# Dzh-16/FLASH-Viterbi

Hardware: AMD Instinct MI355X
Metric: trellis_cells_per_sec (higher is better)
Workload: dtype f32 scores (+f64 add per cell, rounded to f32 as the reference does)

## Files before the change

flash_viterbi_amd/csrc/fv_full.hip:

```cpp
#include "fv_internal.h"
#include "fv_kernels.hip.inc"
#include "flashvit_testing.h"

namespace {

int pick_kernel(const fv_ctx *ctx)
{
    if (ctx->opt_kernel == FV_KERNEL_F64_STREAM) return FV_KERNEL_F64_STREAM;
    if (!ctx->view.logs_nonpositive) return FV_KERNEL_F64_STREAM;
    if (ctx->opt_kernel == FV_KERNEL_F16_REFINE || ctx->opt_kernel == FV_KERNEL_F32_REFINE ||
        ctx->opt_kernel == FV_KERNEL_Q16_REFINE || ctx->opt_kernel == FV_KERNEL_U16_REFINE)
        return ctx->opt_kernel;
    if (ctx->opt_kernel == FV_KERNEL_SPARSE_Q16) return ctx->SPdata.p ? FV_KERNEL_SPARSE_Q16 : FV_KERNEL_U16_REFINE;
    return (ctx->SPdata.p && ctx->density <= 0.35) ? FV_KERNEL_SPARSE_Q16 : FV_KERNEL_U16_REFINE;
}

constexpr int U_UP = 16, U_DB32 = 4, U_DB64 = 2, U_DB16 = 2;

constexpr int nb_slot(int NB) { return NB == 1 ? 0 : NB == 2 ? 1 : NB == 4 ? 2 : 3; }
template <typename TA> constexpr int tab_slot()
{
    return std::is_same<TA, double>::value ? 0 : std::is_same<TA, float>::value ? 1 : std::is_same<TA, fvk::half_t>::value ? 2 : 3;
}
template <typename TA, int NB, bool DB> constexpr unsigned long long step_variant()
{
    return 1ull << ((tab_slot<TA>() == 0 ? 0 : 4 + (tab_slot<TA>() - 1) * 6) + (DB ? 0 : 4) + nb_slot(NB));
}
template <typename TA> constexpr unsigned long long slab_variant() { return 1ull << (22 + tab_slot<TA>()); }
template <int NB, bool DB, int NWV> constexpr unsigned long long u16_variant()
{
    return 1ull << (26 + (NWV == 16 ? 0 : 8) + (DB ? 4 : 0) + nb_slot(NB));
}
template <int NB> constexpr unsigned long long sparse_variant() { return 1ull << (42 + nb_slot(NB)); }
template <int NB, bool MEM> constexpr unsigned long long csr_variant() { return 1ull << (FV_TV_CSR_SHIFT + (MEM ? 4 : 0) + nb_slot(NB)); }
template <int NB, bool MEM> constexpr unsigned long long csr_f64_variant() { return (1ull << (FV_TV_CSR64_SHIFT + nb_slot(NB))) | (MEM ? 1ull << (FV_TV_CSR64_SHIFT + 4) : 0ull); }
static_assert(step_variant<double, 8, true>() == FV_TV_F64_NB8 && step_variant<float, 2, false>() == FV_TV_F32_UP_NB2 &&
              step_variant<fvk::half_t, 1, true>() == FV_TV_F16_NB1 && step_variant<fvk::q16_t, 2, false>() == FV_TV_Q16_UP_NB2 &&
// ... 258 lines not shown
}

int max_batch_for(int nrows, bool u16_only)
{
    if (u16_only) {
        if (fvk::u16_lds_bytes<8, 8>(nrows) <= 160 * 1024) return 8;
        if (fvk::u16_lds_bytes<4, 8>(nrows) <= 160 * 1024) return 4;
        if (fvk::u16_lds_bytes<2, 8>(nrows) <= 160 * 1024) return 2;
        return 1;
    }
    int nb = fvk::MAX_BATCH;
    while (nb > 1) {
        size_t need = nb == 8 ? fvk::step_lds_bytes<8>(nrows) : nb == 4 ? fvk::step_lds_bytes<4>(nrows)
                                                                        : fvk::step_lds_bytes<2>(nrows);
        if (need <= 160 * 1024) break;
        nb >>= 1;
    }
    return nb;
}

struct ProfRange { size_t first, count; };

int prof_event(fv_ctx *ctx, size_t idx, hipEvent_t *out)
{
    while (ctx->prof_events.size() <= idx) {
        hipEvent_t e;
        FV_HIP(hipEventCreate(&e));
        ctx->prof_events.push_back(e);
    }
    *out = ctx->prof_events[idx];
    return 0;
}

enum { BATCH_NONE = 0, BATCH_SERIAL = 1, BATCH_FORK = 2 };
int run_generation_full(fv_ctx *ctx, std::vector<fv::Pass> &passes, int kernel, size_t &nprof, int batch = BATCH_NONE)
{
    const int K = ctx->K;
    const int np = (int)passes.size();
    if (np == 0) return 0;
    std::stable_sort(passes.begin(), passes.end(),
                     [](const fv::Pass &a, const fv::Pass &b) { return a.R - a.L > b.R - b.L; });
    for (int base = 0; base < np; base += fvk::PASS_CHUNK) {
        fvk::PassChunk ch;
        ch.n = std::min(fvk::PASS_CHUNK, np - base);
        for (int q = 0; q < ch.n; ++q) {
            const fv::Pass &p = passes[base + q];
            ch.p[q] = fvk::PassDesc{ p.L, p.R, p.from_pi ? 1 : 0, p.whole ? 1 : 0, (long long)(base + q) * 2 * ctx->nrows };
        }
        if (ctx->csr)
            hipLaunchKernelGGL(fvk::init_rows_csr, dim3((K + 255) / 256, ch.n), dim3(256), 0, ctx->stream, ch, ctx->CRptr.p,
                               ctx->CRcol.p, ctx->CRlog.p, ctx->view.lb64, ctx->LPi64.p, ctx->d_ob.p, ctx->d_ans.p, ctx->d_rows.p, K);
        else
        hipLaunchKernelGGL(fvk::init_rows, dim3((K + 255) / 256, ch.n), dim3(256), 0, ctx->stream, ch,
                           ctx->LA64.p, ctx->nrows, ctx->view.lb64, ctx->LPi64.p, ctx->d_ob.p, ctx->d_ans.p,
                           ctx->d_rows.p, K);
        FV_HIP(hipGetLastError());
    }
    const int maxlen = passes[0].R - passes[0].L;
    const bool slabbed = (kernel == FV_KERNEL_F64_STREAM || kernel == FV_KERNEL_Q16_REFINE) && !ctx->full_ok;
    int cap = std::max(1, std::min(ctx->opt_max_batch, slabbed ? 4 : max_batch_for(ctx->nrows, !ctx->full_ok)));
    if (kernel == FV_KERNEL_SPARSE_CSR || kernel == FV_KERNEL_CSR_F64) cap = ctx->opt_max_batch;
    const bool whole_gen = passes[0].whole;
    constexpr int FORK_STREAMS = 3, FORK_CAP = 4;
    const bool two = ((kernel == FV_KERNEL_U16_REFINE && ctx->u16_ok) || ((kernel == FV_KERNEL_SPARSE_Q16 || kernel == FV_KERNEL_SPARSE_CSR || kernel == FV_KERNEL_CSR_F64) && maxlen >= 64)) &&
                     !(ctx->opt_debug & 262144) && (!whole_gen || batch == BATCH_FORK) && np > FORK_CAP &&
                     !ctx->opt_profile && !(ctx->opt_debug & 64);
    const int nbatches = (np + FORK_CAP - 1) / FORK_CAP;
    const int nstreams = two ? std::min(FORK_STREAMS, nbatches) : 1;
    auto fork = [&]() -> int {
        FV_HIP(hipEventRecord(ctx->ev_fork, ctx->stream));
        for (int q = 1; q < nstreams; ++q) FV_HIP(hipStreamWaitEvent(ctx->aux[q - 1], ctx->ev_fork, 0));
        return 0;
    };
    if (two) {
        cap = std::min(cap, FORK_CAP);
        if (!ctx->fork_active) {
            hipError_t qe;
            while ((qe = hipStreamQuery(ctx->stream)) == hipErrorNotReady) std::this_thread::yield();
            FV_HIP(qe);
        }
        ctx->fork_active = true;
        { int rc = fork(); if (rc) return rc; }
    }
    ctx->forked_batches = two;
    struct Unfork { fv_ctx *c; ~Unfork() { c->forked_batches = false; c->lstream = nullptr; } } unfork{ ctx };
    auto join = [&]() -> int {
        for (int q = 1; q < nstreams; ++q) {
            FV_HIP(hipEventRecord(ctx->ev_join[q - 1], ctx->aux[q - 1]));
            FV_HIP(hipStreamWaitEvent(ctx->stream, ctx->ev_join[q - 1], 0));
        }
        return 0;
    };
    const bool col_last = !(ctx->opt_debug & 8);
    const bool use_graph = (ctx->opt_debug & 64) && !ctx->opt_profile;
    if (use_graph) FV_HIP(hipStreamBeginCapture(ctx->stream, hipStreamCaptureModeThreadLocal));
    if (whole_gen && !use_graph) FV_HIP(hipEventRecord(ctx->ev_s0, ctx->stream));
    int active = np;
    for (int s = 1; s <= maxlen; ++s) {
        while (active > 0 && passes[active - 1].R - passes[active - 1].L < s) --active;
        int full = active;
        if (col_last) while (full > 0 && passes[full - 1].R - passes[full - 1].L == s && !passes[full - 1].whole) --full;
        auto row = [&](int q, int parity) { return ctx->d_rows.p + (size_t)q * 2 * ctx->nrows + (size_t)parity * ctx->nrows; };
        for (int base = 0; base < full; base += cap) {
            const int nb = std::min(cap, full - base);
            fvk::TaskSlot slots[fvk::MAX_BATCH];
            for (int q = 0; q < nb; ++q) {
                const fv::Pass &p = passes[base + q];
                slots[q].t1_in = row(base + q, (s - 1) & 1);
                slots[q].t1_out = row(base + q, s & 1);
                slots[q].tmp_row = ctx->view.lb32 + (size_t)ctx->h_ob[p.L + s] * K;
                slots[q].tmp64_row = ctx->view.lb64 + (size_t)ctx->h_ob[p.L + s] * K;
                slots[q].bp_out = ctx->d_bp.p + (size_t)(p.L + s) * K;
            }
            hipEvent_t e0 = nullptr, e1 = nullptr;
            if (ctx->opt_profile) {
                int rc = prof_event(ctx, nprof, &e0); if (rc) return rc;
                rc = prof_event(ctx, nprof + 1, &e1); if (rc) return rc;
                nprof += 2;
                FV_HIP(hipEventRecord(e0, ctx->stream));
            }
            const int other = two ? (base / cap) % nstreams : 0;
            ctx->lstream = other ? ctx->aux[other - 1] : ctx->stream;
            int rc = launch_step_kernel(ctx, kernel, slots, nb, s & 1);
            ctx->lstream = nullptr;
            if (rc) return rc;
            if (ctx->opt_profile) FV_HIP(hipEventRecord(e1, ctx->stream));
            ctx->stats.step_launches += 1;
            ctx->stats.task_steps += nb;
        }
        for (int sid = 0; sid < nstreams; ++sid) {
            fvk::ColArgs c;
            c.LA64 = ctx->LA64.p; c.ans = ctx->d_ans.p; c.K = K; c.nrows = ctx->nrows; c.n = 0;
            hipStream_t cst = sid ? ctx->aux[sid - 1] : ctx->stream;
            auto flush = [&]() -> int {
                if (c.n == 0) return 0;
                if (ctx->csr) {
                    fvk::CsrColArgs cc;
                    cc.ck = ctx->CSk.p; cc.c64 = ctx->CS64.p; cc.tile_off = ctx->CSoff.p; cc.tile_nwb = ctx->CSnwb.p;
                    cc.ans = ctx->d_ans.p; cc.K = K; cc.n = c.n;
                    std::copy(c.p, c.p + c.n, cc.p);
                    hipLaunchKernelGGL(fvk::last_column_csr, dim3(c.n), dim3(256), 0, cst, cc);
                } else
                hipLaunchKernelGGL(fvk::last_column, dim3(c.n), dim3(256), 0, cst, c);
                FV_HIP(hipGetLastError());
                ctx->stats.column_steps += c.n;
                c.n = 0;
                return 0;
            };
            for (int q = full; q < active; ++q) {
                const int owner = (two && s > 1) ? (q / cap) % nstreams : 0;
                if (owner != sid) continue;
                const fv::Pass &p = passes[q];
                c.p[c.n++] = fvk::ColJob{ row(q, (s - 1) & 1), ctx->view.lb32 + (size_t)ctx->h_ob[p.R] * K, ctx->d_bp.p + (size_t)p.R * K, p.R };
                if (c.n == fvk::COL_CHUNK) { int rc = flush(); if (rc) return rc; }
            }
            int rc = flush();
            if (rc) return rc;
        }
    }
    if (use_graph) {
        hipGraph_t g = nullptr;
        FV_HIP(hipStreamEndCapture(ctx->stream, &g));
        hipGraphExec_t ge = nullptr;
        FV_HIP(hipGraphInstantiate(&ge, g, nullptr, nullptr, 0));
        if (whole_gen) FV_HIP(hipEventRecord(ctx->ev_s0, ctx->stream));
        FV_HIP(hipGraphLaunch(ge, ctx->stream));
        ctx->graphs.push_back(ge);
        (void)hipGraphDestroy(g);
    }
    if (whole_gen && !two) FV_HIP(hipEventRecord(ctx->ev_s1, ctx->stream));
    if (two) { int rc = join(); if (rc) return rc; }
    if (whole_gen && two) FV_HIP(hipEventRecord(ctx->ev_s1, ctx->stream));
    if (batch) {
        fvk::ArgmaxArgs a;
        a.rows = ctx->d_rows.p; a.ans = ctx->d_ans.p; a.score = ctx->d_score.p; a.K = K; a.nrows = ctx->nrows; a.n = 0;
        auto flush = [&]() -> int {
            if (a.n == 0) return 0;
            hipLaunchKernelGGL(fvk::final_argmax_batch, dim3(a.n), dim3(1024), 0, ctx->stream, a);
            FV_HIP(hipGetLastError());
            a.n = 0;
            return 0;
        };
        for (int q = 0; q < np; ++q) {
            if (!passes[q].whole) continue;
            const int len = passes[q].R - passes[q].L;
            a.j[a.n++] = fvk::ArgmaxJob{ q * 2 + (len & 1), passes[q].R, passes[q].seq };
            if (a.n == fvk::ARGMAX_CHUNK) { int rc = flush(); if (rc) return rc; }
        }
        int rc = flush();
        if (rc) return rc;
    }
    for (int q = 0; q < np && !batch; ++q) {
        if (!passes[q].whole) continue;
        const int len = passes[q].R - passes[q].L;
        const float *last = ctx->d_rows.p + (size_t)q * 2 * ctx->nrows + (size_t)(len & 1) * ctx->nrows;
        hipLaunchKernelGGL(fvk::final_argmax, dim3(1), dim3(1024), 0, ctx->stream, last, K,
                           ctx->d_ans.p + passes[q].R, ctx->d_score.p);
        FV_HIP(hipGetLastError());
    }
    for (int base = 0; base < np; base += fvk::PASS_CHUNK) {
        fvk::PassChunk ch;
        ch.n = std::min(fvk::PASS_CHUNK, np - base);
        for (int q = 0; q < ch.n; ++q) {
            const fv::Pass &p = passes[base + q];
            ch.p[q] = fvk::PassDesc{ p.L, p.R, p.from_pi ? 1 : 0, p.whole ? 1 : 0, 0 };
        }
        hipLaunchKernelGGL(fvk::backtrack, dim3(ch.n), dim3(64), 0, ctx->stream, ch, ctx->d_bp.p, K, ctx->d_ans.p);
        FV_HIP(hipGetLastError());
    }
    return 0;
}

}

namespace fvi {

int full_setup(fv_ctx *ctx)
{
    int rc = 0;
    if ((rc = allow_big_lds<float, 1>(ctx)) || (rc = allow_big_lds<float, 2>(ctx)) || (rc = allow_big_lds<float, 4>(ctx)) ||
        (rc = allow_big_lds<float, 8>(ctx)) || (rc = allow_big_lds<double, 1>(ctx)) || (rc = allow_big_lds<double, 2>(ctx)) ||
        (rc = allow_big_lds<double, 4>(ctx)) || (rc = allow_big_lds<double, 8>(ctx)) ||
        (rc = allow_big_lds<fvk::half_t, 1>(ctx)) || (rc = allow_big_lds<fvk::half_t, 2>(ctx)) ||
        (rc = allow_big_lds<fvk::half_t, 4>(ctx)) || (rc = allow_big_lds<fvk::half_t, 8>(ctx)) ||
        (rc = allow_big_lds<fvk::q16_t, 1>(ctx)) || (rc = allow_big_lds<fvk::q16_t, 2>(ctx)) ||
        (rc = allow_big_lds<fvk::q16_t, 4>(ctx)) || (rc = allow_big_lds<fvk::q16_t, 8>(ctx)) ||
        (rc = set_big_lds(ctx, &fvk::trellis_step_sparse<1>)) || (rc = set_big_lds(ctx, &fvk::trellis_step_sparse<2>)) ||
        (rc = set_big_lds(ctx, &fvk::trellis_step_sparse<4>)) || (rc = set_big_lds(ctx, &fvk::trellis_step_sparse<8>)))
        return rc;
    if ((rc = set_big_lds(ctx, &fvk::trellis_step_csr<1, false>)) || (rc = set_big_lds(ctx, &fvk::trellis_step_csr<2, false>)) ||
        (rc = set_big_lds(ctx, &fvk::trellis_step_csr<4, false>)) || (rc = set_big_lds(ctx, &fvk::trellis_step_csr<8, false>)))
        return rc;
// ... 124 lines not shown
        double lmax, dqmax;
        std::memcpy(&lmax, &bits[0], 8); std::memcpy(&dqmax, &bits[1], 8);
        const float stepf = lmax > 0.0 ? (float)(lmax / 65534.0) : 1.0f;
        ctx->windowq = std::nextafter((float)(2.0 * dqmax), HUGE_VALF);
        ctx->qscale = -stepf;
        ctx->laq16_ready = true;
    }
    return fvi::ensure_workspace(ctx, T, rows_needed, nscores);
}

void start_full_stats(fv_ctx *ctx, int kernel, int generations)
{
    long long table = (long long)((ctx->K + fvk::TILE_W - 1) / fvk::TILE_W) * ctx->nrows * fvk::TILE_W * (kernel == FV_KERNEL_F64_STREAM ? 8 : kernel == FV_KERNEL_F32_REFINE ? 4 : 2);
    if (kernel == FV_KERNEL_SPARSE_Q16) table = (long long)ctx->SPdata.bytes();
    if (kernel == FV_KERNEL_SPARSE_CSR) table = (long long)(ctx->CSk.bytes() + ctx->CSq.bytes());
    if (kernel == FV_KERNEL_CSR_F64) table = (long long)(ctx->CSk.bytes() + ctx->CS64.bytes());
    ctx->start_stats(kernel, generations, table, ctx->density);
}

int decode_full_impl(fv_ctx *ctx, const int *ob, int T, int n_split, int mode, int *path_out, float *score_out)
{
    if (!ctx || !path_out || T < 2 || n_split < 1) return FV_ERR_ARG;
    int rc = fvi::emission_view(ctx, ob, T);
    if (rc) return rc;
    if (ctx->K == 0) return FV_ERR_STATE;
    auto t0 = clk::now();
    fv::Plan plan;
    rc = fv::build_plan(T, n_split, mode, ctx->nranks, plan);
    if (rc) return rc;
    size_t most = 1;
    std::vector<std::vector<fv::Pass>> gens = fvi::deal_passes(ctx, plan, &most);
    int kernel = FV_KERNEL_AUTO;
    if ((rc = prepare_full(ctx, ob, T, most, kernel))) return rc;
    start_full_stats(ctx, kernel, plan.generations());

    if ((rc = fvi::begin_decode(ctx, ob, T))) return rc;
    FV_HIP(hipEventRecord(ctx->ev_start, ctx->stream));
    size_t nprof = 0;
    ctx->fork_active = false;
    for (size_t g = 0; g < gens.size(); ++g) {
        ctx->stats.passes += (int)gens[g].size();
        if ((rc = run_generation_full(ctx, gens[g], kernel, nprof))) return rc;
        if (g == 0) FV_HIP(hipEventRecord(ctx->ev_top, ctx->stream));
    }
    ctx->close_stats((long long)ctx->K * ctx->K, ctx->K);
    const long long whole[2] = { 0, T };
    return fvi::finish_decode(ctx, plan, whole, 1, path_out, score_out, nullptr, t0, nprof, false);
}

int decode_full_batch_impl(fv_ctx *ctx, const int *ob, const long long *offsets, int nseq, int n_split, int mode, int *path_out,
                           float *score_out, int *status_out)
{
    const char *who = "fv_decode_full_batch";
    std::vector<int> lengths;
    int rc = fvi::batch_lengths(ctx, who, ob, offsets, nseq, n_split, mode, path_out, lengths);
    if (rc || (rc = fvi::batch_symbols(ctx, who, ob, offsets, nseq))) return rc;
    auto t0 = clk::now();
    const int sumT = (int)offsets[nseq];
    fv::Plan plan;
    if ((rc = fvi::batch_plan(ctx, who, lengths, n_split, mode, plan))) return rc;
    size_t most = 1;
    std::vector<std::vector<fv::Pass>> gens = fvi::deal_passes(ctx, plan, &most);
    int kernel = FV_KERNEL_AUTO;
    if ((rc = prepare_full(ctx, ob, sumT, most, kernel, std::max(nseq, 2)))) return rc;
    start_full_stats(ctx, kernel, plan.generations());

    if ((rc = fvi::begin_decode(ctx, ob, sumT))) return rc;
    FV_HIP(hipEventRecord(ctx->ev_start, ctx->stream));
    size_t nprof = 0;
    ctx->fork_active = false;
    const int gen0 = (ctx->opt_debug & (1 << 28)) ? BATCH_SERIAL : BATCH_FORK;
    for (size_t g = 0; g < gens.size(); ++g) {
        ctx->stats.passes += (int)gens[g].size();
        if ((rc = run_generation_full(ctx, gens[g], kernel, nprof, gen0))) return rc;
        if (g == 0) FV_HIP(hipEventRecord(ctx->ev_top, ctx->stream));
    }
    ctx->close_stats((long long)ctx->K * ctx->K, ctx->K);
    return fvi::finish_decode(ctx, plan, offsets, nseq, path_out, score_out, status_out, t0, nprof, false);
}

int test_forward_impl(fv_ctx *ctx, const int *ob, int T, const fv_test_pass *tp, int np, float *rows_out, int *bp_out,
                      unsigned long long *variants_out)
{
    if (!tp || np < 1 || !rows_out || !bp_out || T < 2) return FV_ERR_ARG;
    if (int rv = fvi::emission_view(ctx, ob, T)) return rv;
    if (ctx->K == 0) return FV_ERR_STATE;
    const int K = ctx->K;
    std::vector<fv::Pass> gen((size_t)np);
    std::vector<int> byL((size_t)np);
    for (int q = 0; q < np; ++q) {
        const fv_test_pass &p = tp[q];
        if (p.L < 0 || p.R <= p.L || p.R >= T) { ctx->detail = "fv_test_forward: a pass needs 0 <= L < R < T"; return FV_ERR_ARG; }
        if (p.L == 0 ? p.init_state >= 0 : (p.init_state < 0 || p.init_state >= K)) {
            ctx->detail = "fv_test_forward: init_state < 0 (Pi) at L = 0 only, a state in [0, K) at L > 0";
            return FV_ERR_ARG;
        }
        gen[(size_t)q] = fv::Pass{ p.L, p.R, p.L == 0, false, 0, -1 };
        byL[(size_t)q] = q;
    }
    std::sort(byL.begin(), byL.end(), [&](int a, int b) { return tp[a].L < tp[b].L; });
    for (int q = 1; q < np; ++q)
        if (tp[byL[q]].L <= tp[byL[q - 1]].R) { ctx->detail = "fv_test_forward: passes overlap"; return FV_ERR_ARG; }
    int kernel = FV_KERNEL_AUTO;
    int rc = prepare_full(ctx, ob, T, (size_t)np, kernel);
    if (rc) return rc;
    start_full_stats(ctx, kernel, 1);
    ctx->stats.passes = np;
// ... 152 lines not shown
```

flash_viterbi_amd/csrc/fv_kernels.hip.inc:

```
#pragma once

#include <hip/hip_runtime.h>

#include <cfloat>
#include <climits>
#include <cstdint>
#include <type_traits>

#include "fv_device_common.h"

#ifdef FV_TIMING_BUILD
#define FV_TIMING_BIT(debug, bit) (((debug) & (bit)) != 0)
#else
#define FV_TIMING_BIT(debug, bit) false
#endif

namespace fvk {


struct TaskSlot {
    const float *t1_in;
    float *t1_out;
    int *bp_out;
    const float *tmp_row;
// ... 1329 lines not shown
        float r = m1[t];
        int kbest = k1[t];
        wave_best(r, kbest);
        if (lane < TILE_W) { redR[(t * TILE_W + c) * SP_WAVES + w] = r; redK[(t * TILE_W + c) * SP_WAVES + w] = kbest; }
    }
    __syncthreads();
    if (w < NB && w < args.nb) {
        float r = FV_NEG_INF;
        int kbest = INT_MAX;
        if (rg < 2) {
            const float4 fv = *reinterpret_cast<const float4 *>(redR + (w * TILE_W + c) * SP_WAVES + rg * 4);
            const int4 fk = *reinterpret_cast<const int4 *>(redK + (w * TILE_W + c) * SP_WAVES + rg * 4);
            r = fv.x; kbest = fk.x;
            if (better(fv.y, fk.y, r, kbest)) { r = fv.y; kbest = fk.y; }
            if (better(fv.z, fk.z, r, kbest)) { r = fv.z; kbest = fk.z; }
            if (better(fv.w, fk.w, r, kbest)) { r = fv.w; kbest = fk.w; }
        }
        wave_best(r, kbest);
        if (lane < TILE_W && col < K) {
            const bool any = r > -FLT_MAX;
            args.t[w].t1_out[col] = any ? r : -FLT_MAX;
            args.t[w].bp_out[col] = any ? kbest : -1;
        }
    }
}

template <int NB>
static inline size_t csr_f64_lds_bytes(int nrows, bool mem)
{
    return (mem ? (size_t)0 : (size_t)nrows * NB * 4) + (size_t)NB * SP_WAVES * TILE_W * 8;
}



__global__ void init_rows(const PassChunk ch, const double *LA64, int nrows, const double *LB64T,
                          const double *LPi64, const int *ob, const int *ans, float *rows, int K)
{
    const PassDesc p = ch.p[blockIdx.y];
    const int i = blockIdx.x * blockDim.x + threadIdx.x;
    if (i >= K) return;
    int st = p.from_pi ? -1 : ans[p.L - 1];
    const double x = st < 0 ? LPi64[i] : LA64[tab_index<4>(st, i, nrows)];
    rows[p.row_off + i] = (float)(x + LB64T[(size_t)ob[p.L] * K + i]);
}

__global__ __launch_bounds__(1024) void final_argmax(const float *row, int K, int *ans_last, float *score_out)
{
    __shared__ float sv[16];
    __shared__ int sk[16];
    float v = FV_NEG_INF;
    int k = INT_MAX;
    for (int i = threadIdx.x; i < K; i += blockDim.x) {
        const float x = row[i];
        if (x > v) { v = x; k = i; }
    }
#pragma unroll
    for (int m = 1; m < 64; m <<= 1) {
        float ov = __shfl_xor(v, m);
        int ok = __shfl_xor(k, m);
        if (better(ov, ok, v, k)) { v = ov; k = ok; }
    }
    const int lane = threadIdx.x & 63, w = threadIdx.x >> 6;
    if (lane == 0) { sv[w] = v; sk[w] = k; }
    __syncthreads();
    if (threadIdx.x == 0) {
        for (int q = 1; q < (int)(blockDim.x >> 6); ++q)
            if (better(sv[q], sk[q], v, k)) { v = sv[q]; k = sk[q]; }
        *ans_last = k;
        *score_out = v;
    }
}

struct ArgmaxJob { int row; int R; int seq; };
constexpr int ARGMAX_CHUNK = 256;
struct ArgmaxArgs { const float *rows; int *ans; float *score; int K, nrows, n; ArgmaxJob j[ARGMAX_CHUNK]; };

// ... 8 lines not shown
    int k = INT_MAX;
    for (int i = threadIdx.x; i < args.K; i += blockDim.x) {
        const float x = row[i];
        if (x > v) { v = x; k = i; }
    }
#pragma unroll
    for (int m = 1; m < 64; m <<= 1) {
        float ov = __shfl_xor(v, m);
        int ok = __shfl_xor(k, m);
        if (better(ov, ok, v, k)) { v = ov; k = ok; }
    }
    const int lane = threadIdx.x & 63, w = threadIdx.x >> 6;
    if (lane == 0) { sv[w] = v; sk[w] = k; }
    __syncthreads();
    if (threadIdx.x == 0) {
        for (int q = 1; q < (int)(blockDim.x >> 6); ++q)
            if (better(sv[q], sk[q], v, k)) { v = sv[q]; k = sk[q]; }
        args.ans[job.R] = k;
        args.score[job.seq] = v;
    }
}

struct ColJob { const float *t1_in; const float *tmp_row; int *bp_row; int R; };
constexpr int COL_CHUNK = 48;
struct ColArgs { const double *LA64; const int *ans; int K, nrows, n; ColJob p[COL_CHUNK]; };

__global__ __launch_bounds__(256) void last_column(const ColArgs args)
{
    __shared__ float sv[4];
    __shared__ int sk[4];
    const ColJob job = args.p[blockIdx.x];
    const int i = args.ans[job.R];
    if (i < 0 || i >= args.K) return;
    const float tmp = job.tmp_row[i];
    const double *col = args.LA64 + (size_t)(i >> 4) * args.nrows * TILE_W + (i & 15) * 4;
    float best = FV_NEG_INF;
    int arg = INT_MAX;
    for (int k0 = threadIdx.x; k0 < args.K; k0 += 256 * 4) {
        float t1[4];
        double L[4];
#pragma unroll
        for (int u = 0; u < 4; ++u) {
            const int k = k0 + 256 * u, ks = k < args.K ? k : 0;
            t1[u] = job.t1_in[ks];
            L[u] = col[(size_t)(ks >> 2) * (TILE_W * 4) + (ks & 3)];
        }
#pragma unroll
        for (int u = 0; u < 4; ++u) {
            const int k = k0 + 256 * u;
            if (k < args.K) {
                const float y = exact_cell(tmp, t1[u], L[u]);
                if (y > best) { best = y; arg = k; }
            }
        }
    }
#pragma unroll
    for (int m = 1; m < 64; m <<= 1) {
        const float ov = __shfl_xor(best, m);
        const int ok = __shfl_xor(arg, m);
        if (better(ov, ok, best, arg)) { best = ov; arg = ok; }
    }
    const int lane = threadIdx.x & 63, w = threadIdx.x >> 6;
    if (lane == 0) { sv[w] = best; sk[w] = arg; }
    __syncthreads();
    if (threadIdx.x == 0) {
        for (int q = 1; q < 4; ++q)
            if (better(sv[q], sk[q], best, arg)) { best = sv[q]; arg = sk[q]; }
        job.bp_row[i] = best > -FLT_MAX ? arg : -1;
    }
}

__global__ void init_rows_csr(const PassChunk ch, const long long *rptr, const int *rcol, const double *rlog,
                              const double *LB64T, const double *LPi64, const int *ob, const int *ans, float *rows, int K)
{
    const PassDesc p = ch.p[blockIdx.y];
    const int i = blockIdx.x * blockDim.x + threadIdx.x;
    if (i >= K) return;
    const int st = p.from_pi ? -1 : ans[p.L - 1];
    double x;
    if (st < 0) {
        x = LPi64[i];
    } else {
        long long lo = rptr[st], hi = rptr[st + 1];
        const long long end = hi;
        while (lo < hi) {
            const long long mid = lo + (hi - lo) / 2;
            if (rcol[mid] < i) lo = mid + 1; else hi = mid;
        }
        x = (lo < end && rcol[lo] == i) ? rlog[lo] : -__builtin_huge_val();
    }
    rows[p.row_off + i] = (float)(x + LB64T[(size_t)ob[p.L] * K + i]);
}

struct CsrColArgs {
    const uint4 *ck; const double *c64; const long long *tile_off; const int *tile_nwb;
    const int *ans; int K, n; ColJob p[COL_CHUNK];
};

__global__ __launch_bounds__(256) void last_column_csr(const CsrColArgs args)
{
    __shared__ float sv[4];
    __shared__ int sk[4];
    const ColJob job = args.p[blockIdx.x];
    const int i = args.ans[job.R];
    if (i < 0 || i >= args.K) return;
    const float tmp = job.tmp_row[i];
    const int tile = i >> 4, c = i & 15;
    const size_t v0 = (size_t)args.tile_off[tile] + c;
    const int nent = args.tile_nwb[tile] * 16;
    const unsigned int *kw = reinterpret_cast<const unsigned int *>(args.ck);
    float best = FV_NEG_INF;
    int arg = INT_MAX;
    for (int n0 = threadIdx.x; n0 < nent; n0 += 256 * 4) {
        float t1[4];
        double L[4];
        int ks[4];
#pragma unroll
        for (int u = 0; u < 4; ++u) {
            const int n = n0 + 256 * u, ns = n < nent ? n : 0;
            const size_t pos = 4 * (v0 + (size_t)(ns >> 2) * TILE_W) + (ns & 3);
            ks[u] = (int)kw[pos];
            L[u] = args.c64[pos];
            t1[u] = job.t1_in[ks[u]];
        }
#pragma unroll
        for (int u = 0; u < 4; ++u) {
            if (n0 + 256 * u < nent) {
                const float y = exact_cell(tmp, t1[u], L[u]);
                if (y > best) { best = y; arg = ks[u]; }
            }
        }
    }
#pragma unroll
    for (int m = 1; m < 64; m <<= 1) {
        const float ov = __shfl_xor(best, m);
        const int ok = __shfl_xor(arg, m);
        if (better(ov, ok, best, arg)) { best = ov; arg = ok; }
    }
    const int lane = threadIdx.x & 63, w = threadIdx.x >> 6;
    if (lane == 0) { sv[w] = best; sk[w] = arg; }
    __syncthreads();
    if (threadIdx.x == 0) {
        for (int q = 1; q < 4; ++q)
            if (better(sv[q], sk[q], best, arg)) { best = sv[q]; arg = sk[q]; }
        job.bp_row[i] = best > -FLT_MAX ? arg : -1;
    }
}

__global__ __launch_bounds__(64) void backtrack(const PassChunk ch, const int *bp, int K, int *ans)
{
    const PassDesc p = ch.p[blockIdx.x];
    const int lane = threadIdx.x, len = p.R - p.L;
    auto hop = [&](int st, int j) { return st >= 0 ? bp[(size_t)j * K + st] : -1; };
    if (len < BT_MIN_PARALLEL) {
        if (lane != 0) return;
        int st = ans[p.R];
        for (int j = p.R; j > p.L; --j) { st = hop(st, j); ans[j - 1] = st; }
        return;
    }
    const int cs = (len + 63) / 64;
    auto top = [&](int c) { return max(p.R - c * cs, p.L); };
    int base = 0, exact = ans[p.R];
    while (base < 64 && top(base) > p.L) {
        int x = -2, y = -2;
        if (lane >= base && top(lane) > p.L) {
            const int t_hi = top(lane), t_lo = top(lane + 1);
            int t = min(top(base), t_hi + BT_WARMUP), st = exact;
            for (; t > t_hi; --t) st = hop(st, t);
            x = st;
            for (; t > t_lo; --t) { st = hop(st, t); ans[t - 1] = st; }
            y = st;
        }
        const int y_above = __shfl_up(y, 1);
        const bool ok = lane <= base || top(lane) <= p.L || min(top(base), top(lane) + BT_WARMUP) == top(base) || x == y_above;
        const unsigned long long bad = ~__ballot(ok);
        if (!bad) break;
        const int f = __ffsll((long long)bad) - 1;
        exact = __shfl(y, f - 1);
        base = f;
    }
}

constexpr int EMIS_BLOCK = 256;
template <typename TIN>
__global__ __launch_bounds__(EMIS_BLOCK) void stage_emissions(const TIN *src, long long ld, int T, int K, float *E32,
                                                              double *E64, unsigned long long *flags)
{
    __shared__ unsigned int s_flags;
    __shared__ unsigned long long s_bad;
    if (threadIdx.x == 0) { s_flags = 0u; s_bad = ~0ull; }
    __syncthreads();
    unsigned int f = 0u;
    unsigned long long bad = ~0ull;
    for (int t = blockIdx.y; t < T; t += gridDim.y) {
        const TIN *row = src + (size_t)t * (size_t)ld;
        for (int i = blockIdx.x * EMIS_BLOCK + threadIdx.x; i < K; i += gridDim.x * EMIS_BLOCK) {
            const double x = (double)row[i];
            const float xf = (float)x;
            const size_t e = (size_t)t * K + i;
            const bool ok = xf < HUGE_VALF && (xf > -HUGE_VALF || x == -HUGE_VAL);
            if (!ok) { f |= 1u; bad = min(bad, (unsigned long long)e); }
            if (x > 0.0) f |= 2u;
            E32[e] = xf;
            E64[e] = x;
        }
    }
    if (f) atomicOr(&s_flags, f);
    if (bad != ~0ull) atomicMin(&s_bad, bad);
    __syncthreads();
    if (threadIdx.x == 0) {
        if (s_flags) atomicOr(&flags[0], (unsigned long long)s_flags);
        if (s_bad != ~0ull) atomicMin(&flags[1], s_bad);
// ... 5 lines not shown
```

Measured before the change: 1027 billion.

## Fuse generation backtrack, child row init and length-one columns into seam kernel

Adds a close_generation kernel that, per parent pass, walks the backtrack chain, resolves the length-one column passes of the next generation inline, and initialises the next generation's child rows. It replaces the separate backtrack, init_rows and last_column launches at generation boundaries. The aim is fewer kernel launches and serial dependencies between generations. In exchange, per-parent blocks of 1024 threads do serial column work, and the CSR row lookup now repeats a binary search per candidate.

```diff
diff --git a/flash_viterbi_amd/csrc/fv_full.hip b/flash_viterbi_amd/csrc/fv_full.hip
--- a/flash_viterbi_amd/csrc/fv_full.hip
+++ b/flash_viterbi_amd/csrc/fv_full.hip
@@ -3,6 +3,11 @@
 #include "flashvit_testing.h"
 
 namespace {
+
+fvk::CsrModel csr_model(const fv_ctx *ctx)
+{
+    return fvk::CsrModel{ ctx->CRptr.p, ctx->CRcol.p, ctx->CRlog.p, ctx->LPi64.p, ctx->CSk.p, ctx->CS64.p, ctx->CSoff.p, ctx->CSnwb.p };
+}
 
 int pick_kernel(const fv_ctx *ctx)
 {
@@ -327,15 +332,121 @@
     return 0;
 }
 
+struct SeamPlan {
+    std::vector<std::vector<fv::Pass>> cols;
+    std::vector<fvk::SeamChunk> open;
+    std::vector<std::vector<fvk::SeamChunk>> close;
+};
+
+struct SeamFamily { int L, R, walk; std::vector<fvk::SeamChild> rows, cols; };
+
+void pack_seam(const std::vector<SeamFamily> &fam, std::vector<fvk::SeamChunk> &out)
+{
+    fvk::SeamChunk ch;
+    int nc = 0;
+    ch.np = 0;
+    auto flush = [&]() { if (ch.np) out.push_back(ch); ch.np = 0; nc = 0; };
+    for (const SeamFamily &f : fam) {
+        size_t r = 0, c = 0;
+        int walk = f.walk;
+        do {
+            if (ch.np == fvk::SEAM_PARENTS || nc == fvk::SEAM_CHILDREN) flush();
+            const int nrow = (int)std::min<size_t>(f.rows.size() - r, (size_t)(fvk::SEAM_CHILDREN - nc));
+            const int ncol = (int)std::min<size_t>(f.cols.size() - c, (size_t)(fvk::SEAM_CHILDREN - nc - nrow));
+            ch.p[ch.np++] = fvk::SeamParent{ f.L, f.R, walk, nc, nrow, ncol };
+            for (int q = 0; q < nrow; ++q) ch.c[nc++] = f.rows[r++];
+            for (int q = 0; q < ncol; ++q) ch.c[nc++] = f.cols[c++];
+            walk = 0;
+        } while (r < f.rows.size() || c < f.cols.size());
+    }
+    flush();
+}
+
+int plan_seams(fv_ctx *ctx, std::vector<std::vector<fv::Pass>> &gens, SeamPlan &sp)
+{
+    const bool col_last = !(ctx->opt_debug & 8);
+    const size_t ng = gens.size();
+    sp.cols.assign(ng, {});
+    sp.close.assign(ng, {});
+    for (size_t g = 0; g < ng; ++g) {
+        std::vector<fv::Pass> &v = gens[g];
+        std::stable_sort(v.begin(), v.end(), [](const fv::Pass &a, const fv::Pass &b) { return a.R - a.L > b.R - b.L; });
+        size_t keep = v.size();
+        while (col_last && g > 0 && keep > 0 && v[keep - 1].R - v[keep - 1].L == 1 && !v[keep - 1].whole) --keep;
+        sp.cols[g].assign(v.begin() + keep, v.end());
+        v.resize(keep);
+    }
+    std::vector<SeamFamily> fam;
+    for (size_t q = 0; ng > 0 && q < gens[0].size(); ++q) {
+        const fv::Pass &p = gens[0][q];
+        fam.push_back(SeamFamily{ p.L, p.R, 0, { fvk::SeamChild{ p.L, p.R, p.from_pi ? 1 : 0, (int)q } }, {} });
+    }
+    pack_seam(fam, sp.open);
+    std::vector<int> byL;
+    for (size_t g = 0; g < ng; ++g) {
+        const std::vector<fv::Pass> &par = gens[g];
+        if (par.empty()) continue;
+        fam.clear();
+        for (const fv::Pass &p : par) fam.push_back(SeamFamily{ p.L, p.R, 1, {}, {} });
+        if (g + 1 < ng) {
+            byL.resize(par.size());
+            for (size_t q = 0; q < par.size(); ++q) byL[q] = (int)q;
+            std::sort(byL.begin(), byL.end(), [&](int a, int b) { return par[a].L < par[b].L; });
+            auto parent_of = [&](const fv::Pass &c) -> SeamFamily * {
+                auto it = std::upper_bound(byL.begin(), byL.end(), c.L, [&](int L, int q) { return L < par[q].L; });
+                if (it == byL.begin()) return nullptr;
+                const fv::Pass &p = par[*(it - 1)];
+                return (c.L > p.L && c.R <= p.R && !c.from_pi) ? &fam[*(it - 1)] : nullptr;
+            };
+            for (size_t q = 0; q < gens[g + 1].size(); ++q) {
+                const fv::Pass &c = gens[g + 1][q];
+                SeamFamily *f = parent_of(c);
+                if (!f) { ctx->detail = "internal: a pass without a parent in the generation before it"; return FV_ERR_STATE; }
+                f->rows.push_back(fvk::SeamChild{ c.L, c.R, 0, (int)q });
+            }
+            for (const fv::Pass &c : sp.cols[g + 1]) {
+                SeamFamily *f = parent_of(c);
+                if (!f) { ctx->detail = "internal: a pass without a parent in the generation before it"; return FV_ERR_STATE; }
+                f->cols.push_back(fvk::SeamChild{ c.L, c.R, 0, -1 });
+            }
+        }
+        pack_seam(fam, sp.close[g]);
+    }
+    return 0;
+}
+
+int launch_seams(fv_ctx *ctx, const std::vector<fvk::SeamChunk> &chunks)
+{
+    for (const fvk::SeamChunk &ch : chunks) {
+        if (ctx->csr) {
+            fvk::SeamArgs<fvk::CsrModel> a;
+            a.m = csr_model(ctx);
+            a.LB64T = ctx->view.lb64; a.LB32T = ctx->view.lb32; a.ob = ctx->d_ob.p; a.bp = ctx->d_bp.p; a.ans = ctx->d_ans.p;
+            a.rows = ctx->d_rows.p; a.K = ctx->K; a.nrows = ctx->nrows;
+            hipLaunchKernelGGL(fvk::close_generation<fvk::CsrModel>, dim3(ch.np), dim3(fvk::SEAM_BLOCK), 0, ctx->stream, a, ch);
+        } else {
+            fvk::SeamArgs<fvk::DenseModel> a;
+            a.m = fvk::DenseModel{ ctx->LA64.p, ctx->LPi64.p, ctx->nrows, ctx->K };
+            a.LB64T = ctx->view.lb64; a.LB32T = ctx->view.lb32; a.ob = ctx->d_ob.p; a.bp = ctx->d_bp.p; a.ans = ctx->d_ans.p;
+            a.rows = ctx->d_rows.p; a.K = ctx->K; a.nrows = ctx->nrows;
+            hipLaunchKernelGGL(fvk::close_generation<fvk::DenseModel>, dim3(ch.np), dim3(fvk::SEAM_BLOCK), 0, ctx->stream, a, ch);
+        }
+        FV_HIP(hipGetLastError());
+    }
+    return 0;
+}
+
 enum { BATCH_NONE = 0, BATCH_SERIAL = 1, BATCH_FORK = 2 };
-int run_generation_full(fv_ctx *ctx, std::vector<fv::Pass> &passes, int kernel, size_t &nprof, int batch = BATCH_NONE)
+int run_generation_full(fv_ctx *ctx, std::vector<fv::Pass> &passes, int kernel, size_t &nprof, int batch = BATCH_NONE,
+                        const std::vector<fvk::SeamChunk> *open = nullptr, const std::vector<fvk::SeamChunk> *close = nullptr)
 {
     const int K = ctx->K;
     const int np = (int)passes.size();
     if (np == 0) return 0;
     std::stable_sort(passes.begin(), passes.end(),
                      [](const fv::Pass &a, const fv::Pass &b) { return a.R - a.L > b.R - b.L; });
-    for (int base = 0; base < np; base += fvk::PASS_CHUNK) {
+    if (open) { int rc = launch_seams(ctx, *open); if (rc) return rc; }
+    for (int base = 0; base < np && !close; base += fvk::PASS_CHUNK) {
         fvk::PassChunk ch;
         ch.n = std::min(fvk::PASS_CHUNK, np - base);
         for (int q = 0; q < ch.n; ++q) {
@@ -343,8 +454,8 @@
             ch.p[q] = fvk::PassDesc{ p.L, p.R, p.from_pi ? 1 : 0, p.whole ? 1 : 0, (long long)(base + q) * 2 * ctx->nrows };
         }
         if (ctx->csr)
-            hipLaunchKernelGGL(fvk::init_rows_csr, dim3((K + 255) / 256, ch.n), dim3(256), 0, ctx->stream, ch, ctx->CRptr.p,
-                               ctx->CRcol.p, ctx->CRlog.p, ctx->view.lb64, ctx->LPi64.p, ctx->d_ob.p, ctx->d_ans.p, ctx->d_rows.p, K);
+            hipLaunchKernelGGL(fvk::init_rows_csr, dim3((K + 255) / 256, ch.n), dim3(256), 0, ctx->stream, ch, csr_model(ctx),
+                               ctx->view.lb64, ctx->d_ob.p, ctx->d_ans.p, ctx->d_rows.p, K);
         else
         hipLaunchKernelGGL(fvk::init_rows, dim3((K + 255) / 256, ch.n), dim3(256), 0, ctx->stream, ch,
                            ctx->LA64.p, ctx->nrows, ctx->view.lb64, ctx->LPi64.p, ctx->d_ob.p, ctx->d_ans.p,
@@ -357,8 +468,12 @@
     if (kernel == FV_KERNEL_SPARSE_CSR || kernel == FV_KERNEL_CSR_F64) cap = ctx->opt_max_batch;
     const bool whole_gen = passes[0].whole;
     constexpr int FORK_STREAMS = 3, FORK_CAP = 4;
+    constexpr long long FORK_MIN_STEPS = 0;
+    const bool col_last = !(ctx->opt_debug & 8);
+    long long full_steps = 0;
+    for (const fv::Pass &p : passes) full_steps += p.R - p.L - ((col_last && !p.whole) ? 1 : 0);
     const bool two = ((kernel == FV_KERNEL_U16_REFINE && ctx->u16_ok) || ((kernel == FV_KERNEL_SPARSE_Q16 || kernel == FV_KERNEL_SPARSE_CSR || kernel == FV_KERNEL_CSR_F64) && maxlen >= 64)) &&
-                     !(ctx->opt_debug & 262144) && (!whole_gen || batch == BATCH_FORK) && np > FORK_CAP &&
+                     !(ctx->opt_debug & 262144) && (!whole_gen || batch == BATCH_FORK) && np > FORK_CAP && full_steps >= FORK_MIN_STEPS &&
                      !ctx->opt_profile && !(ctx->opt_debug & 64);
     const int nbatches = (np + FORK_CAP - 1) / FORK_CAP;
     const int nstreams = two ? std::min(FORK_STREAMS, nbatches) : 1;
@@ -386,7 +501,6 @@
         }
         return 0;
     };
-    const bool col_last = !(ctx->opt_debug & 8);
     const bool use_graph = (ctx->opt_debug & 64) && !ctx->opt_profile;
     if (use_graph) FV_HIP(hipStreamBeginCapture(ctx->stream, hipStreamCaptureModeThreadLocal));
     if (whole_gen && !use_graph) FV_HIP(hipEventRecord(ctx->ev_s0, ctx->stream));
@@ -431,7 +545,7 @@
                 if (c.n == 0) return 0;
                 if (ctx->csr) {
                     fvk::CsrColArgs cc;
-                    cc.ck = ctx->CSk.p; cc.c64 = ctx->CS64.p; cc.tile_off = ctx->CSoff.p; cc.tile_nwb = ctx->CSnwb.p;
+                    cc.m = csr_model(ctx);
                     cc.ans = ctx->d_ans.p; cc.K = K; cc.n = c.n;
                     std::copy(c.p, c.p + c.n, cc.p);
                     hipLaunchKernelGGL(fvk::last_column_csr, dim3(c.n), dim3(256), 0, cst, cc);
@@ -493,6 +607,7 @@
                            ctx->d_ans.p + passes[q].R, ctx->d_score.p);
         FV_HIP(hipGetLastError());
     }
+    if (close) return launch_seams(ctx, *close);
     for (int base = 0; base < np; base += fvk::PASS_CHUNK) {
         fvk::PassChunk ch;
         ch.n = std::min(fvk::PASS_CHUNK, np - base);
@@ -683,6 +798,8 @@
     std::vector<std::vector<fv::Pass>> gens = fvi::deal_passes(ctx, plan, &most);
     int kernel = FV_KERNEL_AUTO;
     if ((rc = prepare_full(ctx, ob, T, most, kernel))) return rc;
+    SeamPlan seams;
+    if ((rc = plan_seams(ctx, gens, seams))) return rc;
     start_full_stats(ctx, kernel, plan.generations());
 
     if ((rc = fvi::begin_decode(ctx, ob, T))) return rc;
@@ -690,8 +807,10 @@
     size_t nprof = 0;
     ctx->fork_active = false;
     for (size_t g = 0; g < gens.size(); ++g) {
-        ctx->stats.passes += (int)gens[g].size();
-        if ((rc = run_generation_full(ctx, gens[g], kernel, nprof))) return rc;
+        ctx->stats.passes += (int)(gens[g].size() + seams.cols[g].size());
+        ctx->stats.column_steps += (int)seams.cols[g].size();
+        if (gens[g].empty()) continue;
+        if ((rc = run_generation_full(ctx, gens[g], kernel, nprof, BATCH_NONE, g == 0 ? &seams.open : nullptr, &seams.close[g]))) return rc;
         if (g == 0) FV_HIP(hipEventRecord(ctx->ev_top, ctx->stream));
     }
     ctx->close_stats((long long)ctx->K * ctx->K, ctx->K);
@@ -714,6 +833,8 @@
     std::vector<std::vector<fv::Pass>> gens = fvi::deal_passes(ctx, plan, &most);
     int kernel = FV_KERNEL_AUTO;
     if ((rc = prepare_full(ctx, ob, sumT, most, kernel, std::max(nseq, 2)))) return rc;
+    SeamPlan seams;
+    if ((rc = plan_seams(ctx, gens, seams))) return rc;
     start_full_stats(ctx, kernel, plan.generations());
 
     if ((rc = fvi::begin_decode(ctx, ob, sumT))) return rc;
@@ -722,8 +843,10 @@
     ctx->fork_active = false;
     const int gen0 = (ctx->opt_debug & (1 << 28)) ? BATCH_SERIAL : BATCH_FORK;
     for (size_t g = 0; g < gens.size(); ++g) {
-        ctx->stats.passes += (int)gens[g].size();
-        if ((rc = run_generation_full(ctx, gens[g], kernel, nprof, gen0))) return rc;
+        ctx->stats.passes += (int)(gens[g].size() + seams.cols[g].size());
+        ctx->stats.column_steps += (int)seams.cols[g].size();
+        if (gens[g].empty()) continue;
+        if ((rc = run_generation_full(ctx, gens[g], kernel, nprof, gen0, g == 0 ? &seams.open : nullptr, &seams.close[g]))) return rc;
         if (g == 0) FV_HIP(hipEventRecord(ctx->ev_top, ctx->stream));
     }
     ctx->close_stats((long long)ctx->K * ctx->K, ctx->K);
diff --git a/flash_viterbi_amd/csrc/fv_kernels.hip.inc b/flash_viterbi_amd/csrc/fv_kernels.hip.inc
--- a/flash_viterbi_amd/csrc/fv_kernels.hip.inc
+++ b/flash_viterbi_amd/csrc/fv_kernels.hip.inc
@@ -1385,6 +1385,81 @@
 }
 
 
+struct DenseModel {
+    const double *LA64, *LPi64; int nrows, K;
+    __device__ __forceinline__ double row_at(int st, int i) const { return st < 0 ? LPi64[i] : LA64[tab_index<4>(st, i, nrows)]; }
+    __device__ __forceinline__ int count(int) const { return K; }
+    __device__ __forceinline__ void cand(int i, int n, int &k, double &L) const
+    {
+        k = n;
+        L = LA64[(size_t)(i >> 4) * nrows * TILE_W + (i & 15) * 4 + (size_t)(n >> 2) * (TILE_W * 4) + (n & 3)];
+    }
+};
+struct CsrModel {
+    const long long *rptr; const int *rcol; const double *rlog, *LPi64;
+    const uint4 *ck; const double *c64; const long long *tile_off; const int *tile_nwb;
+    __device__ __forceinline__ double row_at(int st, int i) const
+    {
+        if (st < 0) return LPi64[i];
+        long long lo = rptr[st], hi = rptr[st + 1];
+        const long long end = hi;
+        while (lo < hi) {
+            const long long mid = lo + (hi - lo) / 2;
+            if (rcol[mid] < i) lo = mid + 1; else hi = mid;
+        }
+        return (lo < end && rcol[lo] == i) ? rlog[lo] : -__builtin_huge_val();
+    }
+    __device__ __forceinline__ int count(int i) const { return tile_nwb[i >> 4] * 16; }
+    __device__ __forceinline__ void cand(int i, int n, int &k, double &L) const
+    {
+        const size_t pos = 4 * ((size_t)tile_off[i >> 4] + (i & 15) + (size_t)(n >> 2) * TILE_W) + (n & 3);
+        k = (int)reinterpret_cast<const unsigned int *>(ck)[pos];
+        L = c64[pos];
+    }
+};
+
+__device__ __forceinline__ float init_cell(double x, double logb) { return (float)(x + logb); }
+
+template <int NT, class Model, class Score>
+__device__ __forceinline__ int best_predecessor(const Model &m, int i, float tmp, Score t1, float *sv, int *sk)
+{
+    const int count = m.count(i);
+    float best = FV_NEG_INF;
+    int arg = INT_MAX;
+    for (int n0 = threadIdx.x; n0 < count; n0 += NT * 4) {
+        float t[4];
+        double L[4];
+        int ks[4];
+#pragma unroll
+        for (int u = 0; u < 4; ++u) {
+            const int n = n0 + NT * u;
+            m.cand(i, n < count ? n : 0, ks[u], L[u]);
+            t[u] = t1(ks[u]);
+        }
+#pragma unroll
+        for (int u = 0; u < 4; ++u) {
+            if (n0 + NT * u < count) {
+                const float y = exact_cell(tmp, t[u], L[u]);
+                if (y > best) { best = y; arg = ks[u]; }
+            }
+        }
+    }
+#pragma unroll
+    for (int mk = 1; mk < 64; mk <<= 1) {
+        const float ov = __shfl_xor(best, mk);
+        const int ok = __shfl_xor(arg, mk);
+        if (better(ov, ok, best, arg)) { best = ov; arg = ok; }
+    }
+    const int lane = threadIdx.x & 63, w = threadIdx.x >> 6;
+    if (lane == 0) { sv[w] = best; sk[w] = arg; }
+    __syncthreads();
+    if (threadIdx.x == 0) {
+        for (int q = 1; q < NT / 64; ++q)
+            if (better(sv[q], sk[q], best, arg)) { best = sv[q]; arg = sk[q]; }
+    }
+    return best > -FLT_MAX ? arg : -1;
+}
+
 
 __global__ void init_rows(const PassChunk ch, const double *LA64, int nrows, const double *LB64T,
                           const double *LPi64, const int *ob, const int *ans, float *rows, int K)
@@ -1392,9 +1467,8 @@
     const PassDesc p = ch.p[blockIdx.y];
     const int i = blockIdx.x * blockDim.x + threadIdx.x;
     if (i >= K) return;
-    int st = p.from_pi ? -1 : ans[p.L - 1];
-    const double x = st < 0 ? LPi64[i] : LA64[tab_index<4>(st, i, nrows)];
-    rows[p.row_off + i] = (float)(x + LB64T[(size_t)ob[p.L] * K + i]);
+    const int st = p.from_pi ? -1 : ans[p.L - 1];
+    rows[p.row_off + i] = init_cell(DenseModel{ LA64, LPi64, nrows, K }.row_at(st, i), LB64T[(size_t)ob[p.L] * K + i]);
 }
 
 __global__ __launch_bounds__(1024) void final_argmax(const float *row, int K, int *ans_last, float *score_out)
@@ -1469,70 +1543,21 @@
     const ColJob job = args.p[blockIdx.x];
     const int i = args.ans[job.R];
     if (i < 0 || i >= args.K) return;
-    const float tmp = job.tmp_row[i];
-    const double *col = args.LA64 + (size_t)(i >> 4) * args.nrows * TILE_W + (i & 15) * 4;
-    float best = FV_NEG_INF;
-    int arg = INT_MAX;
-    for (int k0 = threadIdx.x; k0 < args.K; k0 += 256 * 4) {
-        float t1[4];
-        double L[4];
-#pragma unroll
-        for (int u = 0; u < 4; ++u) {
-            const int k = k0 + 256 * u, ks = k < args.K ? k : 0;
-            t1[u] = job.t1_in[ks];
-            L[u] = col[(size_t)(ks >> 2) * (TILE_W * 4) + (ks & 3)];
-        }
-#pragma unroll
-        for (int u = 0; u < 4; ++u) {
-            const int k = k0 + 256 * u;
-            if (k < args.K) {
-                const float y = exact_cell(tmp, t1[u], L[u]);
-                if (y > best) { best = y; arg = k; }
-            }
-        }
-    }
-#pragma unroll
-    for (int m = 1; m < 64; m <<= 1) {
-        const float ov = __shfl_xor(best, m);
-        const int ok = __shfl_xor(arg, m);
-        if (better(ov, ok, best, arg)) { best = ov; arg = ok; }
-    }
-    const int lane = threadIdx.x & 63, w = threadIdx.x >> 6;
-    if (lane == 0) { sv[w] = best; sk[w] = arg; }
-    __syncthreads();
-    if (threadIdx.x == 0) {
-        for (int q = 1; q < 4; ++q)
-            if (better(sv[q], sk[q], best, arg)) { best = sv[q]; arg = sk[q]; }
-        job.bp_row[i] = best > -FLT_MAX ? arg : -1;
-    }
-}
-
-__global__ void init_rows_csr(const PassChunk ch, const long long *rptr, const int *rcol, const double *rlog,
-                              const double *LB64T, const double *LPi64, const int *ob, const int *ans, float *rows, int K)
+    const int arg = best_predecessor<256>(DenseModel{ args.LA64, nullptr, args.nrows, args.K }, i, job.tmp_row[i],
+                                          [&](int k) { return job.t1_in[k]; }, sv, sk);
+    if (threadIdx.x == 0) job.bp_row[i] = arg;
+}
+
+__global__ void init_rows_csr(const PassChunk ch, const CsrModel m, const double *LB64T, const int *ob, const int *ans, float *rows, int K)
 {
     const PassDesc p = ch.p[blockIdx.y];
     const int i = blockIdx.x * blockDim.x + threadIdx.x;
     if (i >= K) return;
     const int st = p.from_pi ? -1 : ans[p.L - 1];
-    double x;
-    if (st < 0) {
-        x = LPi64[i];
-    } else {
-        long long lo = rptr[st], hi = rptr[st + 1];
-        const long long end = hi;
-        while (lo < hi) {
-            const long long mid = lo + (hi - lo) / 2;
-            if (rcol[mid] < i) lo = mid + 1; else hi = mid;
-        }
-        x = (lo < end && rcol[lo] == i) ? rlog[lo] : -__builtin_huge_val();
-    }
-    rows[p.row_off + i] = (float)(x + LB64T[(size_t)ob[p.L] * K + i]);
-}
-
-struct CsrColArgs {
-    const uint4 *ck; const double *c64; const long long *tile_off; const int *tile_nwb;
-    const int *ans; int K, n; ColJob p[COL_CHUNK];
-};
+    rows[p.row_off + i] = init_cell(m.row_at(st, i), LB64T[(size_t)ob[p.L] * K + i]);
+}
+
+struct CsrColArgs { CsrModel m; const int *ans; int K, n; ColJob p[COL_CHUNK]; };
 
 __global__ __launch_bounds__(256) void last_column_csr(const CsrColArgs args)
 {
@@ -1541,53 +1566,14 @@
     const ColJob job = args.p[blockIdx.x];
     const int i = args.ans[job.R];
     if (i < 0 || i >= args.K) return;
-    const float tmp = job.tmp_row[i];
-    const int tile = i >> 4, c = i & 15;
-    const size_t v0 = (size_t)args.tile_off[tile] + c;
-    const int nent = args.tile_nwb[tile] * 16;
-    const unsigned int *kw = reinterpret_cast<const unsigned int *>(args.ck);
-    float best = FV_NEG_INF;
-    int arg = INT_MAX;
-    for (int n0 = threadIdx.x; n0 < nent; n0 += 256 * 4) {
-        float t1[4];
-        double L[4];
-        int ks[4];
-#pragma unroll
-        for (int u = 0; u < 4; ++u) {
-            const int n = n0 + 256 * u, ns = n < nent ? n : 0;
-            const size_t pos = 4 * (v0 + (size_t)(ns >> 2) * TILE_W) + (ns & 3);
-            ks[u] = (int)kw[pos];
-            L[u] = args.c64[pos];
-            t1[u] = job.t1_in[ks[u]];
-        }
-#pragma unroll
-        for (int u = 0; u < 4; ++u) {
-            if (n0 + 256 * u < nent) {
-                const float y = exact_cell(tmp, t1[u], L[u]);
-                if (y > best) { best = y; arg = ks[u]; }
-            }
-        }
-    }
-#pragma unroll
-    for (int m = 1; m < 64; m <<= 1) {
-        const float ov = __shfl_xor(best, m);
-        const int ok = __shfl_xor(arg, m);
-        if (better(ov, ok, best, arg)) { best = ov; arg = ok; }
-    }
-    const int lane = threadIdx.x & 63, w = threadIdx.x >> 6;
-    if (lane == 0) { sv[w] = best; sk[w] = arg; }
-    __syncthreads();
-    if (threadIdx.x == 0) {
-        for (int q = 1; q < 4; ++q)
-            if (better(sv[q], sk[q], best, arg)) { best = sv[q]; arg = sk[q]; }
-        job.bp_row[i] = best > -FLT_MAX ? arg : -1;
-    }
-}
-
-__global__ __launch_bounds__(64) void backtrack(const PassChunk ch, const int *bp, int K, int *ans)
-{
-    const PassDesc p = ch.p[blockIdx.x];
-    const int lane = threadIdx.x, len = p.R - p.L;
+    const int arg = best_predecessor<256>(args.m, i, job.tmp_row[i], [&](int k) { return job.t1_in[k]; }, sv, sk);
+    if (threadIdx.x == 0) job.bp_row[i] = arg;
+}
+
+__device__ __forceinline__ void walk_chain(int L, int R, const int *bp, int K, int *ans, int lane)
+{
+    struct { int L, R; } p{ L, R };
+    const int len = p.R - p.L;
     auto hop = [&](int st, int j) { return st >= 0 ? bp[(size_t)j * K + st] : -1; };
     if (len < BT_MIN_PARALLEL) {
         if (lane != 0) return;
@@ -1615,6 +1601,75 @@
         const int f = __ffsll((long long)bad) - 1;
         exact = __shfl(y, f - 1);
         base = f;
+    }
+}
+
+__global__ __launch_bounds__(64) void backtrack(const PassChunk ch, const int *bp, int K, int *ans)
+{
+    const PassDesc p = ch.p[blockIdx.x];
+    walk_chain(p.L, p.R, bp, K, ans, threadIdx.x);
+}
+
+struct SeamParent { int L, R, walk, c0, nrow, ncol; };
+struct SeamChild { int L, R, from_pi, slot; };
+constexpr int SEAM_PARENTS = 40, SEAM_CHILDREN = 128, SEAM_BLOCK = 1024;
+struct SeamChunk { int np; SeamParent p[SEAM_PARENTS]; SeamChild c[SEAM_CHILDREN]; };
+template <class Model>
+struct SeamArgs {
+    Model m;
+    const double *LB64T; const float *LB32T; const int *ob; int *bp; int *ans; float *rows;
+    int K, nrows;
+};
+
+template <class Model>
+__global__ __launch_bounds__(SEAM_BLOCK) void close_generation(const SeamArgs<Model> args, const SeamChunk ch)
+{
+    __shared__ float sv[SEAM_BLOCK / 64];
+    __shared__ int sk[SEAM_BLOCK / 64];
+    __shared__ int s_st[SEAM_CHILDREN], s_ob[SEAM_CHILDREN];
+    const SeamParent P = ch.p[blockIdx.x];
+    const int K = args.K;
+    if (P.walk && threadIdx.x < 64) walk_chain(P.L, P.R, args.bp, K, args.ans, threadIdx.x);
+    __syncthreads();
+    for (int q = threadIdx.x; q < P.nrow + P.ncol; q += SEAM_BLOCK) {
+        const SeamChild C = ch.c[P.c0 + q];
+        s_st[q] = C.from_pi ? -1 : args.ans[C.L - 1];
+        s_ob[q] = args.ob[C.L];
+    }
+    __syncthreads();
+    for (int q = P.nrow; q < P.nrow + P.ncol; ++q) {
+        const SeamChild C = ch.c[P.c0 + q];
+        const int i = args.ans[C.R];
+        int arg = -1;
+        if (i >= 0 && i < K) {
+            const int st = s_st[q];
+            const double *logb = args.LB64T + (size_t)s_ob[q] * K;
+            arg = best_predecessor<SEAM_BLOCK>(args.m, i, args.LB32T[(size_t)args.ob[C.R] * K + i],
+                                               [&](int k) { return init_cell(args.m.row_at(st, k), logb[k]); }, sv, sk);
+            if (threadIdx.x == 0) args.bp[(size_t)C.R * K + i] = arg;
+        }
+        if (threadIdx.x == 0) args.ans[C.L] = arg;
+        __syncthreads();
+    }
+    float *__restrict__ rows = args.rows;
+    const int total = P.nrow * K;
+    for (int e0 = threadIdx.x; e0 < total; e0 += SEAM_BLOCK * 8) {
+        double x[8], b[8];
+#pragma unroll
+        for (int u = 0; u < 8; ++u) {
+            const int e = e0 + SEAM_BLOCK * u, es = e < total ? e : 0;
+            const int q = es / K, i = es - q * K;
+            x[u] = args.m.row_at(s_st[q], i);
+            b[u] = args.LB64T[(size_t)s_ob[q] * K + i];
+        }
+#pragma unroll
+        for (int u = 0; u < 8; ++u) {
+            const int e = e0 + SEAM_BLOCK * u;
+            if (e < total) {
+                const int q = e / K, i = e - q * K;
+                rows[(size_t)ch.c[P.c0 + q].slot * 2 * args.nrows + i] = init_cell(x[u], b[u]);
+            }
+        }
     }
 }
 
```

After: 1043 billion, median of 6. 1.02x the previous value.
